# syguan96/DynaBOA

Hardware: AMD Instinct MI355X
Metric: adapted frames/sec, whole job (3 inner + 1 outer step, bs=1 per sequence, first-order; synthetic 224x224 stream, no 3DPW assets in the image: PA-MPJPE on 3DPW not measured) (higher is better)
Workload: dtype f32

## Files before the change

### dynaboa_amd/csrc/adapt_step.hip

```cpp
#include <math.h>
#include <stdlib.h>
#include <string.h>

#include <algorithm>
#include <atomic>
#include <chrono>
#include <condition_variable>
#include <mutex>
#include <string>
#include <thread>
#include <vector>

#include "dyb_common.h"

extern "C" {
size_t dyb_hmr_param_floats(const void*);
size_t dyb_hmr_act_floats(const void*);
size_t dyb_hmr_workspace_bytes(const void*);
int dyb_hmr_forward_train(void*, const float*, const float*, const float*, int, float*, void*, size_t, unsigned long long, unsigned long long, float,
                          hipStream_t);
long long dyb_hmr_act_offset_rotmat(const void*);
long long dyb_hmr_act_offset_state(const void*);
size_t dyb_lbs_saved_floats(int);
size_t dyb_lbs_bwd_workspace_bytes(int);
// ... 233 lines not shown
  bool adam_prepared = false;
  float pre_ss[DYB_MAX_REPLICAS], pre_bc[DYB_MAX_REPLICAS];
  float *gt_rot = nullptr, *gt_verts[3] = {}, *gt_joints = nullptr, *gt_saved = nullptr, *gt17[2] = {};
  DybEvents* ev = nullptr;
  hipEvent_t e_theta = nullptr, e_side = nullptr, e_gt = nullptr;
  int upd_overlap = 1;
  int par_passes = 1, par_max_replicas = DYB_MAX_REPLICAS;
  hipStream_t par_stream[2] = {nullptr, nullptr};
  hipEvent_t par_ev[8] = {nullptr, nullptr, nullptr, nullptr, nullptr, nullptr, nullptr, nullptr};
  bool out_in_main = false;
  int share_dyn_fwd = 1;
  int upd_blocks = 0;
  hipEvent_t e_upd = nullptr;
  DybFwdGates gates{};
  bool gates_pending = false;
  int upd_late = 1;
  struct LateUpd {
    Stepper* S = nullptr;
    bool adam = false, ema = false;
    const float *g2 = nullptr, *g3 = nullptr;
    const float* p = nullptr;
    float* out = nullptr;
    hipStream_t aux = nullptr;
    DybRep scope{};
    float ss[DYB_MAX_REPLICAS], bc[DYB_MAX_REPLICAS];
  } late;
  size_t grp_bounds[2] = {0, 0};
  bool side_pending = false;
  struct Tail {
    bool on = false;
// ... 108 lines not shown
  Stepper* S = new Stepper();
  S->plan = plan; S->B = B; S->H = H; S->W = W;
  S->n_params = dyb_hmr_param_floats(plan);
  S->act_floats = dyb_hmr_act_floats(plan);
  S->ws_bytes = dyb_hmr_workspace_bytes(plan);
  S->off_rot = (size_t)dyb_hmr_act_offset_rotmat(plan);
  S->off_state = (size_t)dyb_hmr_act_offset_state(plan);
  S->lbs_saved = dyb_lbs_saved_floats(B);
  S->lbs_wsb = dyb_lbs_bwd_workspace_bytes(B);
  S->ev = dyb_hmr_events_create(plan);
  dyb_hmr_param_groups(plan, S->grp_bounds);
  if (const char* e = getenv("DYB_UPD_OVERLAP")) S->upd_overlap = atoi(e);
  if (const char* e = getenv("DYB_UPD_BLOCKS")) S->upd_blocks = atoi(e);
  if (const char* e = getenv("DYB_SHARE_DYN_FWD")) S->share_dyn_fwd = atoi(e);
  if (const char* e = getenv("DYB_UPD_LATE")) S->upd_late = atoi(e);
  if (const char* e = getenv("DYB_FUSE_FAST")) S->fuse_fast = atoi(e);
  if (const char* e = getenv("DYB_FUSE_ADAM")) S->fuse_adam = atoi(e);
  if (const char* e = getenv("DYB_FUSE_EMA")) S->fuse_ema = atoi(e);
  if (const char* e = getenv("DYB_PAR_PASSES")) S->par_passes = atoi(e);
  if (const char* e = getenv("DYB_PAR_MAX_REPLICAS")) S->par_max_replicas = atoi(e);
  if (!S->ev || hipEventCreateWithFlags(&S->e_theta, hipEventDisableTiming) != hipSuccess ||
      hipEventCreateWithFlags(&S->e_side, hipEventDisableTiming) != hipSuccess ||
      hipEventCreateWithFlags(&S->e_gt, hipEventDisableTiming) != hipSuccess ||
      hipEventCreateWithFlags(&S->e_upd, hipEventDisableTiming) != hipSuccess ||
      hipEventCreateWithFlags(&S->gates.ev[0], hipEventDisableTiming) != hipSuccess ||
      hipEventCreateWithFlags(&S->gates.ev[1], hipEventDisableTiming) != hipSuccess ||
      hipEventCreateWithFlags(&S->gates.mid, hipEventDisableTiming) != hipSuccess) {
    delete S;
    return DYB_ERR_LAUNCH;
  }
  *out = S;
  return DYB_OK;
}
extern "C" void dyb_stepper_destroy(void* stepper) {
  Stepper* S = reinterpret_cast<Stepper*>(stepper);
  if (!S) return;
  side_shutdown(*S);
  dyb_hmr_events_destroy(S->ev);
  if (S->e_theta) (void)hipEventDestroy(S->e_theta);
  if (S->e_side) (void)hipEventDestroy(S->e_side);
  if (S->e_gt) (void)hipEventDestroy(S->e_gt);
  if (S->e_upd) (void)hipEventDestroy(S->e_upd);
// ... 8 lines not shown
extern "C" int dyb_stepper_set_i(void* stepper, const char* key, long long v) {
  Stepper* S = reinterpret_cast<Stepper*>(stepper);
  DYB_REQUIRE(S && key, DYB_ERR_ARG);
  const std::string k(key);
  if (k == "n_iter") S->n_iter = (int)v;
  else if (k == "inner_step") S->inner_step = (int)v;
  else if (k == "eval_lower") S->eval_lower = (int)v;
  else if (k == "use_side") S->use_side = (int)v;
  else if (k == "upd_overlap") S->upd_overlap = (int)v;
  else if (k == "side_thread") S->side_thread = (int)v;
  else if (k == "upd_blocks") S->upd_blocks = (int)v;
  else if (k == "share_dyn_fwd") S->share_dyn_fwd = (int)v;
  else if (k == "par_passes") S->par_passes = (int)v;
  else if (k == "par_max_replicas") S->par_max_replicas = (int)v;
  else if (k == "upd_late") S->upd_late = (int)v;
  else if (k == "fuse_fast") { DYB_REQUIRE(!S->bound, DYB_ERR_ARG); S->fuse_fast = (int)v; }
  else if (k == "fuse_adam") S->fuse_adam = (int)v;
  else if (k == "fuse_ema") S->fuse_ema = (int)v;
  else if (k == "metrics") S->metrics = (int)v;
  else if (k == "adam_step") {
    S->adam_t = v;
    for (int r = 0; r < DYB_MAX_REPLICAS; ++r) S->adam_t_rep[r] = v;
  }
  else if (k.compare(0, 10, "adam_step_") == 0) {
    const int r = atoi(k.c_str() + 10);
    DYB_REQUIRE(r >= 0 && r < DYB_MAX_REPLICAS, DYB_ERR_ARG);
    S->adam_t_rep[r] = v;
    if (v > S->adam_t) S->adam_t = v;
  }
  else if (k == "full") S->full = (int)v;
// ... 94 lines not shown
  if (k == "loss_floats") return (S->full ? 16 : 4) * (long long)(S->inner_step + 1 + (S->full && S->dynamic ? S->optim_steps : 0));
  if (k == "slots_per_frame") return (S->eval_lower ? S->inner_step : 0) + 1 + (S->full && S->dynamic ? S->optim_steps : 0);
  return -1;
}
extern "C" double dyb_stepper_get_f(const void* stepper, const char* key) {
  const Stepper* S = reinterpret_cast<const Stepper*>(stepper);
  if (!S || !key) return -1.0;
  const std::string k(key);
  if (k == "host_ms_forward") return S->h_fwd;
  if (k == "host_ms_backward") return S->h_bwd;
  if (k == "host_ms_head") return S->h_head;
  if (k == "host_ms_update") return S->h_update;
  if (k == "host_ms_tail") return S->h_tail;
  if (k == "host_ms_total") return S->h_total;
  if (k == "host_frames") return (double)S->h_frames;
  return -1.0;
}
extern "C" size_t dyb_stepper_workspace_bytes(void* stepper) {
  Stepper* S = reinterpret_cast<Stepper*>(stepper);
  if (!S) return 0;
  Stepper tmp = *S;
  return a64(carve(tmp, nullptr) / 4) * 4 * (size_t)S->nrep;
}
extern "C" int dyb_stepper_bind_workspace(void* stepper, void* ws, size_t bytes, hipStream_t st) {
  Stepper* S = reinterpret_cast<Stepper*>(stepper);
  DYB_REQUIRE(S && ws, DYB_ERR_ARG);
  S->blob = a64(carve(*S, nullptr) / 4) * 4;
  DYB_REQUIRE(bytes >= S->blob * (size_t)S->nrep, DYB_ERR_WORKSPACE);
  S->wsp = reinterpret_cast<char*>(ws);
  S->wsp_bytes = bytes;
// ... 39 lines not shown
    }
  }
  DYB_REQUIRE(S.inner_step >= 0 && S.inner_step <= 16 && S.n_iter >= 1 && S.n_iter <= 3, DYB_ERR_UNSUPPORTED);
  return DYB_OK;
}

static int settle_update(Stepper& S, hipStream_t st);
static int pass_forward(Stepper& S, Pass& P, const float* theta, const float* image, hipStream_t st, bool chain = true) {
  const DybFwdGates* gates = (chain && S.gates_pending) ? &S.gates : nullptr;
  {
    const int rc = dyb_hmr_forward_plain(S.plan, theta, image, S.init_state, S.n_iter, P.acts, P.ws, S.ws_bytes, st, gates);
    if (rc != DYB_OK) {
      if (gates) (void)settle_update(S, st);
      return rc;
    }
    if (gates) { DYB_REQUIRE(!S.gates.late, DYB_ERR_LAUNCH); S.gates_pending = false; }
  }
  const float* rot = P.acts + S.off_rot;
  const float* state = P.acts + S.off_state;
  return dyb_lbs_fwd(S.smpl_f[0], S.smpl_i[0], state + 144, STATE_LD, rot, P.verts, P.joints, P.saved, S.B, st);
}
static int pass_frame_head(Stepper& S, Pass& P, const float* kp2d, hipStream_t st) {
  const float* rot = P.acts + S.off_rot;
  const float* state = P.acts + S.off_state;
  return dyb_frame_losses(rot, state + 144, STATE_LD, state + 154, STATE_LD, P.joints, kp2d, S.gmm_means, S.gmm_prec, S.gmm_logw,
                          (float)S.w2d, (float)S.wshape, (float)S.wpose, P.losses, P.drot_l, P.dshape_l, 10, P.dcam_l, 3, P.djoints_l,
                          S.B, P.lws, (size_t)S.B * 16, st);
}
static int pass_backward(Stepper& S, Pass& P, const float* theta, float* grads, hipStream_t st, hipStream_t aux) {
  RUN(dyb_scale_add(nullptr, P.djoints_l, nullptr, P.djoints, (size_t)S.B * NJ * 3, st));
  RUN(dyb_lbs_bwd(S.smpl_f[0], S.smpl_i[0], P.acts + S.off_rot, P.saved, P.djoints, nullptr, P.drot_s, P.dbetas_s, 10, S.B, P.lbs_ws,
                  S.lbs_wsb, st));
  RUN(dyb_head_grad_combine(nullptr, P.drot_l, P.drot_s, nullptr, P.dshape_l, P.dbetas_s, nullptr, P.dcam_l, nullptr, P.d_rot,
                            P.d_state, S.B, st));
  return dyb_hmr_backward_ev(S.plan, theta, P.acts, P.d_rot, P.d_state, S.n_iter, grads, P.ws, S.ws_bytes, st, aux, S.ev);
}
static int gt_meshes(Stepper& S, const float* gt_pose, const float* gt_betas, hipStream_t st) {
  RUN(dyb_rodrigues_fwd(gt_pose, S.gt_rot, S.B * 24, st));
  for (int g = 0; g < 3; ++g)
    RUN(dyb_lbs_fwd(S.smpl_f[g], S.smpl_i[g], gt_betas, 10, S.gt_rot, S.gt_verts[g], S.gt_joints, S.gt_saved, S.B, st));
  RUN(dyb_regress_joints(S.j_h36m, S.gt_verts[1], S.gt17[0], 17, S.B, st));
  return dyb_regress_joints(S.j_h36m, S.gt_verts[2], S.gt17[1], 17, S.B, st);
}
static int record_metrics(Stepper& S, Pass& P, const long long* gender, int slot, hipStream_t st) {
  DYB_REQUIRE(slot >= 0 && slot < S.record_capacity, DYB_ERR_ARG);
  RUN(dyb_regress_joints(S.j_h36m, P.verts, P.pred17, 17, S.B, st));
  float* rec = S.records + (size_t)slot * a64((size_t)S.B * 85 + 1);
  const DybRep& Rp = dyb_rep_current();
  hipLaunchKernelGGL(metric_record_kernel, dim3(1, 1, Rp.n), dim3(256), 0, st, P.pred17, S.gt17[0], S.gt17[1], gender, S.j14, P.verts,
                     S.gt_verts[0], rec, S.B, Rp);
// ... 201 lines not shown
      const double t = (double)(++S.adam_t_rep[r]);
      ss[r] = (float)(S.lr / (1.0 - pow(S.beta1, t)));
      bc[r] = (float)sqrt(1.0 - pow(S.beta2, t));
      if (S.adam_t_rep[r] > S.adam_t) S.adam_t = S.adam_t_rep[r];
    }
  }
  auto range = [&](size_t lo, size_t hi, hipStream_t s) -> int {
    if (adam) {
      const bool fe = ema && S.fuse_ema;
      RUN(adam_range(S, g2, g3, ss, bc, lo, hi, s, fe));
      if (ema && !fe) RUN(dyb_ema_update(S.teacher + lo, S.theta + lo, (float)S.alpha, hi - lo, s));
      return DYB_OK;
    }
    return fastweight_range(S, p, out, g2, g3, lo, hi, s);
  };
  const bool ranged = S.upd_overlap && S.nrep > 1 && aux && aux != st && S.grp_bounds[0] > 0 && S.grp_bounds[1] > S.grp_bounds[0] &&
                      S.grp_bounds[1] < S.n_params;
  if (!ranged) return range(0, S.n_params, st);
  RUN(range(0, S.grp_bounds[0], st));
  HIPOK(hipEventRecord(S.e_upd, st));
  HIPOK(hipStreamWaitEvent(aux, S.e_upd, 0));
  {
    DybStreamCapScope cap(S.upd_blocks > 0 ? (S.upd_blocks / R.n > 0 ? S.upd_blocks / R.n : 1) : 0);
    RUN(range(S.grp_bounds[0], S.grp_bounds[1], aux));
    HIPOK(hipEventRecord(S.gates.ev[0], aux));
    if (S.upd_late) {
      S.late.S = &S; S.late.adam = adam; S.late.ema = ema; S.late.p = p; S.late.out = out; S.late.aux = aux; S.late.scope = R;
      S.late.g2 = g2; S.late.g3 = g3;
      for (int r = 0; r < DYB_MAX_REPLICAS; ++r) { S.late.ss[r] = ss[r]; S.late.bc[r] = bc[r]; }
      S.gates.late = &late_update;
      S.gates.user = &S;
    } else {
      S.gates.late = nullptr;
      RUN(range(S.grp_bounds[1], S.n_params, aux));
      HIPOK(hipEventRecord(S.gates.ev[1], aux));
    }
  }
  S.gates_pending = true;
  return DYB_OK;
}
static int settle_update(Stepper& S, hipStream_t st) {
  if (!S.gates_pending) return DYB_OK;
  if (S.gates.late) {
    HIPOK(hipEventRecord(S.gates.mid, st));
    RUN(late_update(&S));
  }
  HIPOK(hipStreamWaitEvent(st, S.gates.ev[0], 0));
  HIPOK(hipStreamWaitEvent(st, S.gates.ev[1], 0));
  S.gates_pending = false;
  return DYB_OK;
}
static int adam_scope(Stepper& S, hipStream_t st) { return weight_update(S, true, nullptr, nullptr, st, nullptr); }
static int adapt_frame_impl(Stepper& S, const float* image, const float* kp2d, const float* gt_pose, const float* gt_betas,
                            const long long* gender, int record_slot, int loss_slot, hipStream_t st, hipStream_t aux,
                            hipStream_t side) {
  const bool metrics = S.metrics != 0;
  DYB_REQUIRE(!metrics || (gt_pose && gt_betas && gender), DYB_ERR_ARG);
  S.out_in_main = false;
  if (!S.use_side || side == st) side = nullptr;
  const int K = S.inner_step;
  const size_t n = S.n_params;
  float* losslog = (S.loss_log && loss_slot >= 0 && loss_slot < S.loss_capacity) ? S.loss_log + (size_t)loss_slot * 4 * (K + 1) : nullptr;
  int slot = record_slot;
// ... 74 lines not shown
  RUN(pass_forward(S, S.fin, S.theta, image, st));
  RUN(settle_update(S, st));
  if (metrics) RUN(record_metrics(S, S.fin, gender, slot++, st));
  return DYB_OK;
}
static int pass_backward_ext(Stepper& S, Pass& P, const float* theta, float* grads, bool frame_loss, const float* e_rot,
                             const float* e_shape, const float* e_cam, const float* e_joints, hipStream_t st, hipStream_t aux) {
  const size_t nj = (size_t)S.B * NJ * 3;
  if (frame_loss) RUN(dyb_scale_add(nullptr, P.djoints_l, e_joints, P.djoints, nj, st));
  else RUN(dyb_scale_add(nullptr, e_joints, nullptr, P.djoints, nj, st));
  RUN(dyb_lbs_bwd(S.smpl_f[0], S.smpl_i[0], P.acts + S.off_rot, P.saved, P.djoints, nullptr, P.drot_s, P.dbetas_s, 10, S.B, P.lbs_ws,
                  S.lbs_wsb, st));
  const float* z = S.zeros;
  RUN(dyb_head_grad_combine(nullptr, frame_loss ? P.drot_l : z, P.drot_s, e_rot, frame_loss ? P.dshape_l : z, P.dbetas_s, e_shape,
                            frame_loss ? P.dcam_l : z, e_cam, P.d_rot, P.d_state, S.B, st));
  return dyb_hmr_backward_ev(S.plan, theta, P.acts, P.d_rot, P.d_state, S.n_iter, grads, P.ws, S.ws_bytes, st, aux, S.ev);
}
enum { IN_IMAGE = 0, IN_KP, IN_GT_POSE, IN_GT_BETAS, IN_GENDER, IN_HIST_IMAGE, IN_HIST_KP, IN_EX_IMG, IN_EX_KP, IN_EX_POSE,
       IN_EX_BETAS, IN_EX_POSE3D, IN_COUNT };
static int stage_inputs(Stepper& S, const void* const* src, int ld, int k0, int nk, hipStream_t st);
struct FullCtx {
  const void* in[IN_COUNT];
  float* losslog;
  int level_row;
};
struct ParTailGuard {
  hipStream_t st, sB, sC;
  hipEvent_t eB, eC;
  bool armed;
  ~ParTailGuard() {
    if (!armed) return;
// ... 21 lines not shown
    sB = S.par_stream[0]; sC = S.par_stream[1];
    HIPOK(hipEventRecord(S.par_ev[0], st));
    if (motion) HIPOK(hipStreamWaitEvent(sB, S.par_ev[0], 0));
    if (label) HIPOK(hipStreamWaitEvent(sC, S.par_ev[0], 0));
  }
  ParTailGuard tails{st, sB, sC, S.par_ev[6], S.par_ev[7], par};
  if (!have_fwd) RUN(pass_forward(S, P, cur, image, st));
  RUN(pass_frame_head(S, P, kp, st));
  const float* rot = P.acts + S.off_rot;
  const float* state = P.acts + S.off_state;
  if (ranged_before) {
    DYB_REQUIRE(!S.gates_pending && !S.gates.late, DYB_ERR_LAUNCH);
    for (int k = 0; k < 2; ++k) {
      if (motion) HIPOK(hipStreamWaitEvent(sB, S.gates.ev[k], 0));
      if (label) HIPOK(hipStreamWaitEvent(sC, S.gates.ev[k], 0));
    }
  }
  if (par && motion) {
    RUN(pass_forward(S, S.hist, cur, (const float*)C.in[IN_HIST_IMAGE], sB, false));
    HIPOK(hipEventRecord(S.par_ev[1], sB));
  }
  auto label_pass_forward_and_term = [&](hipStream_t s, bool chain) -> int {
    RUN(pass_forward(S, S.ex, cur, (const float*)C.in[IN_EX_IMG], s, chain));
    RUN(dyb_rodrigues_fwd((const float*)C.in[IN_EX_POSE], S.ex_rot, B * 24, s));
    const float* es = S.ex.acts + S.off_state;
    return dyb_aux_loss_terms(2, B, 0, (float)S.label_w, S.ex.acts + S.off_rot, es + 144, STATE_LD, es + 154, STATE_LD, S.ex.joints, nullptr,
                              nullptr, 0, nullptr, 0, nullptr, (const float*)C.in[IN_EX_KP], nullptr, S.ex_rot,
                              (const float*)C.in[IN_EX_BETAS], (const float*)C.in[IN_EX_POSE3D], S.vals_l, S.exg_rot, S.exg_shape, S.exg_cam,
                              S.exg_joints, nullptr, nullptr, s);
  };
// ... 341 lines not shown
  if (S.side_pending) HIPOK(hipStreamWaitEvent(gst, S.e_side, 0));
  RUN(stage_inputs(S, inputs, n, IN_IMAGE, 5, gst));
  const bool have_gt = inputs[2 * n + act[0]] && inputs[3 * n + act[0]] && inputs[4 * n + act[0]];
  if (S.use_side && side && side != st) {
    HIPOK(hipEventRecord(S.e_gt, st));
    HIPOK(hipStreamWaitEvent(side, S.e_gt, 0));
  }
  return adapt_frame_impl(S, S.in_stage[0], S.in_stage[1], have_gt ? S.in_stage[2] : nullptr, have_gt ? S.in_stage[3] : nullptr,
                          have_gt ? reinterpret_cast<const long long*>(S.in_stage[4]) : nullptr, record_slot, loss_slot, st, aux, side);
}
extern "C" int dyb_stepper_join(void* stepper, hipStream_t st) {
  Stepper* S = reinterpret_cast<Stepper*>(stepper);
  DYB_REQUIRE(S, DYB_ERR_ARG);
  RUN(side_wait(*S));
  if ((S->tail.on || S->gtjob.on) && S->tail_stream) RUN(issue_side_work(*S, S->tail_stream));
  if (S->side_pending) {
    HIPOK(hipStreamWaitEvent(st, S->e_side, 0));
    S->side_pending = false;
  }
  return DYB_OK;
}
extern "C" const float* dyb_stepper_output(const void* stepper, int which) {
  const Stepper* S = reinterpret_cast<const Stepper*>(stepper);
  if (!S || !S->bound) return nullptr;
  const Pass& F = (S->out_in_main ? S->main : S->fin);
  switch (which) {
    case 0: return F.acts + S->off_rot;
    case 1: return F.acts + S->off_state;
    case 2: return F.verts;
    case 3: return F.joints;
// ... 4 lines not shown
```

### dynaboa_amd/csrc/dyb_common.h

```cpp
#pragma once
#if defined(__HIP_DEVICE_COMPILE__) && !defined(__gfx950__)
#error "libdynaboa_hip is written for gfx950 (MI355X) only"
#endif
#include <hip/hip_runtime.h>
#include <stdint.h>

#include <vector>
#include "dyb_switches.h"

#define DYB_OK 0
#define DYB_ERR_ARG (-1)
#define DYB_ERR_LAUNCH (-2)
#define DYB_ERR_UNSUPPORTED (-3)
#define DYB_ERR_WORKSPACE (-4)

#define DYB_GN_GROUPS 4
#define DYB_GN_EPS 1e-5f

#define DYB_CHECK_LAUNCH()                                  \
  do {                                                      \
    if (hipGetLastError() != hipSuccess) return DYB_ERR_LAUNCH; \
  } while (0)

#define DYB_REQUIRE(cond, code) \
// ... 217 lines not shown
                       const float* stats, const float* gamma, const float* beta, float* dm, float* dy, float* dgamma, float* dbeta,
                       int HW, int C, int relu, int k, float* part, unsigned* ctr, hipStream_t st);
int dyb_zero_words(unsigned* p, int n, hipStream_t st);
int dyb_gn_bwd_apply_dy(const float* dm, const float* y, const float* stats, const float* part, int nch, int ncolb,
                        const float* gamma, float* dy, float* dgamma, float* dbeta, int N, int HW, int C, hipStream_t st);
int dyb_conv_dgrad_plain_raw(const ConvDesc& d, const float* dy, const float* w, float* dx, const float* addend, void* ws,
                             size_t ws_bytes, int* nslabs, hipStream_t st);
int dyb_conv_wgrad_plain(const ConvDesc& d, const float* x, const float* y_prev, const float* stats_prev, const float* gamma_prev,
                         const float* beta_prev, const float* dy, float* dw, void* ws, size_t ws_bytes, hipStream_t st);
int dyb_avgpool_fwd_tail(const float* x, float* const* dsts, int ndst, int ld, int N, int HW, int C, const float* tail,
                         int tail_ld, int tail_cols, int tail_dst_col, hipStream_t st);

struct DybEvents {
  std::vector<hipEvent_t> dy;
  hipEvent_t join = nullptr;
};
DybEvents* dyb_hmr_events_create(const void* plan);
void dyb_hmr_events_destroy(DybEvents* e);
struct DybFwdGates {
  hipEvent_t ev[2];
  hipEvent_t mid = nullptr;
  int (*late)(void* user) = nullptr;
  void* user = nullptr;
};
void dyb_hmr_param_groups(const void* plan, size_t bounds[2]);
int dyb_hmr_forward_plain(void* plan, const float* params, const float* image, const float* init_state, int n_iter, float* acts,
                          void* ws, size_t ws_bytes, hipStream_t st, const DybFwdGates* gates = nullptr);
int dyb_hmr_backward_ev(void* plan, const float* params, const float* acts, const float* d_rotmat, const float* d_state,
                        int n_iter, float* grads, void* ws, size_t ws_bytes, hipStream_t st, hipStream_t aux, const DybEvents* ev);
```

### dynaboa_amd/csrc/hmr_engine.hip

```cpp
#include <stdlib.h>
#include <string.h>

#include <mutex>
#include <string>
#include <unordered_map>
#include <vector>

#include "dyb_common.h"

extern "C" {
size_t dyb_conv2d_workspace_bytes(int, int, int, int, int, int, int, int, int);
size_t dyb_groupnorm_workspace_bytes(int, int, int);
int dyb_conv2d_nhwc_fwd_gnstats(const float*, const float*, int, const float*, const float*, int, float*, const float*, float*,
                                float*, int*, int, int, int, int, int, int, int, int, int, void*, size_t, hipStream_t);
int dyb_groupnorm_apply_n(const float*, const float*, int, const float*, const float*, const float*, const float*, int,
                          const float*, const float*, float*, float*, float*, int, int, int, int, hipStream_t);
int dyb_conv2d_nhwc_wgrad_gn_n(const float*, const float*, const float*, const float*, const float*, const float*, const float*,
                               const float*, const float*, int, int, const float*, float*, float*, float*, int, int, int, int,
                               int, int, int, int, int, void*, size_t, hipStream_t);
size_t dyb_groupnorm_bwd_partial_floats(int, int, int);
int dyb_conv2d_nhwc_dgrad_gn(const float*, const float*, const float*, const float*, const float*, const float*, float*,
                             const float*, int, int, int, int, int, int, int, int, int, void*, size_t, hipStream_t);
int dyb_conv2d_nhwc_wgrad_gn(const float*, const float*, const float*, const float*, const float*, const float*, float*,
                             float*, float*, int, int, int, int, int, int, int, int, int, void*, size_t, hipStream_t);
// ... 248 lines not shown
  RUN_RC(fill_events(P, P.ev));
  P.events_ready = true;
  return DYB_OK;
}
DybEvents* dyb_hmr_events_create(const void* plan) {
  const HmrPlan* P = reinterpret_cast<const HmrPlan*>(plan);
  if (!P) return nullptr;
  DybEvents* e = new DybEvents();
  if (fill_events(*P, *e) != DYB_OK) { delete e; return nullptr; }
  return e;
}
void dyb_hmr_events_destroy(DybEvents* e) {
  if (!e) return;
  for (hipEvent_t x : e->dy) (void)hipEventDestroy(x);
  (void)hipEventDestroy(e->join);
  delete e;
}
extern "C" size_t dyb_hmr_param_floats(const void* plan) { return reinterpret_cast<const HmrPlan*>(plan)->n_params; }
extern "C" size_t dyb_hmr_act_floats(const void* plan) { return reinterpret_cast<const HmrPlan*>(plan)->act_floats; }
extern "C" size_t dyb_hmr_workspace_bytes(const void* plan) { return reinterpret_cast<const HmrPlan*>(plan)->ws_total; }
extern "C" int dyb_hmr_num_tensors(const void* plan) { return (int)reinterpret_cast<const HmrPlan*>(plan)->tensors.size(); }
extern "C" int dyb_hmr_tensor_info(const void* plan, int i, char* name, int name_cap, int* kind, long long* offset,
                                   int* dims4, int* cin_pad) {
  const HmrPlan* P = reinterpret_cast<const HmrPlan*>(plan);
  DYB_REQUIRE(P && i >= 0 && i < (int)P->tensors.size() && name && kind && offset && dims4 && cin_pad, DYB_ERR_ARG);
  const TensorInfo& t = P->tensors[i];
  strncpy(name, t.name.c_str(), name_cap - 1);
  name[name_cap - 1] = 0;
  *kind = t.kind; *offset = (long long)t.offset; *cin_pad = t.cin_pad;
  for (int k = 0; k < 4; ++k) dims4[k] = t.dims[k];
// ... 210 lines not shown
                            nullptr, nullptr, acts + stem.out, acts + stem.stats, B, stem.Ho * stem.Wo, stem.K, 1, st));
  RUN(dyb_maxpool3x3s2_fwd(acts + stem.out, acts + P.a_pool, reinterpret_cast<uint32_t*>(acts + P.a_poolidx), B, stem.Ho,
                           stem.Wo, stem.K, st));
  const float* x = acts + P.a_pool;
  for (int bi = 0; bi < (int)P.blocks.size(); ++bi) {
    const BlockL& b = P.blocks[bi];
    const ConvL &c1 = P.convs[b.c1], &c2 = P.convs[b.c2], &c3 = P.convs[b.c3];
    if (gates) {
      if (bi == P.layer_last_block[1] + 1) {
        if (gates->ev[0] && hipStreamWaitEvent(st, gates->ev[0], 0) != hipSuccess) return DYB_ERR_LAUNCH;
        if (gates->late) {
          if (gates->mid && hipEventRecord(gates->mid, st) != hipSuccess) return DYB_ERR_LAUNCH;
          RUN(gates->late(gates->user));
        }
      }
      if (bi == P.layer_last_block[2] + 1 && gates->ev[1] && hipStreamWaitEvent(st, gates->ev[1], 0) != hipSuccess) return DYB_ERR_LAUNCH;
    }
    RUN(conv_stats(P, c1, params, acts, x, nullptr, nullptr, 0, w.gn[0], &nA, w, st));
    RUN(conv_stats(P, c2, params, acts, nullptr, &c1, w.gn[0], nA, w.gn[1], &nB, w, st));
    if (b.cd >= 0) RUN(conv_stats(P, P.convs[b.cd], params, acts, x, nullptr, nullptr, 0, w.gn[2], &nD, w, st));
    RUN(conv_stats(P, c3, params, acts, nullptr, &c2, w.gn[1], nB, w.gn[0], &nA, w, st));
    if (b.cd >= 0) {
      const ConvL& cd = P.convs[b.cd];
      RUN(dyb_groupnorm_apply_n(acts + c3.y, w.gn[0], nA, params + c3.gam, params + c3.bet, acts + cd.y, w.gn[2], nD,
                                params + cd.gam, params + cd.bet, acts + cd.stats, acts + c3.out, acts + c3.stats, B,
                                c3.Ho * c3.Wo, c3.K, 1, st));
    } else {
      RUN(dyb_groupnorm_apply_n(acts + c3.y, w.gn[0], nA, params + c3.gam, params + c3.bet, x, nullptr, 0, nullptr, nullptr,
                                nullptr, acts + c3.out, acts + c3.stats, B, c3.Ho * c3.Wo, c3.K, 1, st));
    }
    x = acts + c3.out;
  }
  float* dsts[MAX_ITER];
  for (int t = 0; t < n_iter; ++t) dsts[t] = acts + P.a_xc[t];
  RUN(dyb_avgpool_fwd_tail(x, dsts, n_iter, FC1_IN_PAD, B, P.featHW, FEAT, init_state, STATE_LD, STATE_LD, FEAT, st));
  float* fc1_pre = reinterpret_cast<float*>(w.lin);
  RUN(dyb_linear_fwd(acts + P.a_xc[0], FC1_IN_PAD, params + P.fc1_w, FC1_IN_PAD, params + P.fc1_b, nullptr, 0, fc1_pre, HID, B, FEAT, HID, st));
  for (int t = 0; t < n_iter; ++t) {
    const float* xc = acts + P.a_xc[t];
    RUN(dyb_linear_fwd(xc + FEAT, FC1_IN_PAD, params + P.fc1_w + FEAT, FC1_IN_PAD, nullptr, fc1_pre, HID, acts + P.a_h1[t], HID, B,
                       FC1_IN_PAD - FEAT, HID, st));
    const float* h1 = acts + P.a_h1[t];
    if (drop.on) {
      RUN(dropout_launch(h1, acts + P.a_h1d[t], B * HID, drop, 2u * t, st));
      h1 = acts + P.a_h1d[t];
    }
    RUN(dyb_linear_fwd(h1, HID, params + P.fc2_w, HID, params + P.fc2_b, nullptr, 0, acts + P.a_h2[t], HID, B, HID, HID, st));
    const float* h2 = acts + P.a_h2[t];
    if (drop.on) {
// ... 75 lines not shown
                              acts + c.stats, params + c.gam, params + c.bet, dm, part, P.B, c.Ho * c.Wo, c.K, relu, st,
                              tp ? nullptr : done));
  if (tp) {
    float* dyl = w.dy2 + c.dy;
    RUN(dyb_gn_bwd_apply_dy(dm, acts + c.y, acts + c.stats, part, 0, 0, params + c.gam, dyl, grads + c.gam, grads + c.bet, P.B,
                            c.Ho * c.Wo, c.K, st));
    if (done && hipEventRecord(done, st) != hipSuccess) return DYB_ERR_LAUNCH;
    j.dy = dyl;
  }
  if (jobs) jobs->push_back(j);
  else RUN(run_wgrad(P, j, params, acts, grads, w, w.conv, st));
  *dm_out = dm;
  return DYB_OK;
}
static int flush_wgrads(HmrPlan& P, std::vector<WgradJob>& jobs, hipEvent_t done, const float* params, const float* acts,
                        float* grads, const WsCarve& w, hipStream_t aux) {
  if (hipStreamWaitEvent(aux, done, 0) != hipSuccess) return DYB_ERR_LAUNCH;
  for (const WgradJob& j : jobs) RUN(run_wgrad(P, j, params, acts, grads, w, w.conv_aux, aux));
  jobs.clear();
  return DYB_OK;
}
static int layer_dgrad(HmrPlan& P, int ci, const float* params, const float* acts, const float* dm, float* dx_buf,
                       const float* addend, Pending* out, const WsCarve& w, hipStream_t st, const BwdState& bs) {
  const ConvL& c = P.convs[ci];
  ConvDesc d{P.B, c.H, c.W, c.C, c.K, c.R, c.S, c.stride, c.pad};
  GnBwdSrc src{dm, acts + c.y, acts + c.stats, w.gnb + c.gnb, params + c.gam, bs.nch[ci], bs.ncolb[ci]};
  int ns = 1;
  if (dyb_throughput_mode(P.B))
    RUN(dyb_conv_dgrad_plain_raw(d, w.dy2 + c.dy, params + c.w, dx_buf, addend, w.conv, P.ws_conv,
                                 (out && P.fold_in_reduce) ? &ns : nullptr, st));
  else
    RUN(dyb_conv_dgrad_gn_raw(d, src, params + c.w, dx_buf, addend, w.conv, P.ws_conv, (out && P.fold_in_reduce) ? &ns : nullptr,
                              st));
// ... 10 lines not shown
  ConvDesc d{P.B, c.H, c.W, c.C, c.K, c.R, c.S, c.stride, c.pad};
  *done = false;
  if (!dyb_conv_dgrad_k4_ok(d)) return DYB_OK;
  GnBwdSrc src{dm, acts + c.y, acts + c.stats, w.gnb + c.gnb, params + c.gam, bs.nch[ci], bs.ncolb[ci]};
  int nch = 0, ncolb = 0;
  RUN(dyb_conv_dgrad_k4(d, src, params + c.w, addend, acts + p.y, p.has_out ? acts + p.out : nullptr, acts + p.stats,
                        params + p.gam, params + p.bet, w.dy + p.dy, w.gnb + p.gnb, &nch, &ncolb, st, nullptr));
  bs.nch[pi] = nch; bs.ncolb[pi] = ncolb; bs.reduced[pi] = 1;
  *dm_p = w.dy + p.dy;
  *done = true;
  return DYB_OK;
}

static int backward_body(HmrPlan& P, const float* params, const float* acts, const float* d_rotmat, const float* d_state,
                         int n_iter, float* grads, const WsCarve& w, hipStream_t st, hipStream_t aux, const DybEvents& E,
                         const DropCfg& drop = kNoDrop);

int dyb_hmr_backward_ev(void* plan, const float* params, const float* acts, const float* d_rotmat, const float* d_state,
                        int n_iter, float* grads, void* ws, size_t ws_bytes, hipStream_t st, hipStream_t aux, const DybEvents* ev) {
  HmrPlan* Pp = reinterpret_cast<HmrPlan*>(plan);
  DYB_REQUIRE(Pp && params && acts && d_rotmat && d_state && grads && ws, DYB_ERR_ARG);
  DYB_REQUIRE(n_iter >= 1 && n_iter <= MAX_ITER, DYB_ERR_UNSUPPORTED);
  DYB_REQUIRE(ws_bytes >= Pp->ws_total, DYB_ERR_WORKSPACE);
  if (aux == st || !ev) aux = nullptr;
  WsCarve w = carve(*Pp, ws);
  static const DybEvents none;
  return backward_body(*Pp, params, acts, d_rotmat, d_state, n_iter, grads, w, st, aux, ev ? *ev : none);
}
void dyb_hmr_param_groups(const void* plan, size_t bounds[2]) {
  const HmrPlan* P = reinterpret_cast<const HmrPlan*>(plan);
  bounds[0] = P->convs[P->blocks[P->layer_last_block[1] + 1].c1].w;
  bounds[1] = P->convs[P->blocks[P->layer_last_block[2] + 1].c1].w;
}
int dyb_hmr_forward_plain(void* plan, const float* params, const float* image, const float* init_state, int n_iter, float* acts,
                          void* ws, size_t ws_bytes, hipStream_t st, const DybFwdGates* gates) {
  HmrPlan* Pp = reinterpret_cast<HmrPlan*>(plan);
  DYB_REQUIRE(Pp && params && image && init_state && acts && ws, DYB_ERR_ARG);
  DYB_REQUIRE(n_iter >= 1 && n_iter <= MAX_ITER, DYB_ERR_UNSUPPORTED);
  DYB_REQUIRE(ws_bytes >= Pp->ws_total && Pp->featHW == 49, DYB_ERR_WORKSPACE);
  WsCarve w = carve(*Pp, ws);
  RUN(dyb_nchw3_to_nhwc4(image, acts + Pp->a_x4, Pp->B, Pp->H, Pp->W, st));
  return forward_body(*Pp, params, init_state, n_iter, acts, w, st, kNoDrop, gates);
// ... 32 lines not shown
  DYB_REQUIRE(Pp && params && acts && d_rotmat && d_state && grads && ws, DYB_ERR_ARG);
  DYB_REQUIRE(n_iter >= 1 && n_iter <= MAX_ITER, DYB_ERR_UNSUPPORTED);
  HmrPlan& P = *Pp;
  DYB_REQUIRE(ws_bytes >= P.ws_total, DYB_ERR_WORKSPACE);
  if (aux == st) aux = nullptr;
  if (aux) RUN(ensure_events(P));
  WsCarve w = carve(P, ws);
  GKey key{{(uintptr_t)params, (uintptr_t)acts, (uintptr_t)d_rotmat, (uintptr_t)d_state, (uintptr_t)grads, (uintptr_t)ws,
            (uintptr_t)st, (uintptr_t)aux, (uintptr_t)n_iter, 0}};
  return run_cached(P, P.gbwd, key, st,
                    [&]() { return backward_body(P, params, acts, d_rotmat, d_state, n_iter, grads, w, st, aux, P.ev); });
}

static int backward_body(HmrPlan& P, const float* params, const float* acts, const float* d_rotmat, const float* d_state,
                         int n_iter, float* grads, const WsCarve& w, hipStream_t st, hipStream_t aux, const DybEvents& E,
                         const DropCfg& drop) {
  DybBf16Scope bf(P.bf16 != 0);
  const int B = P.B;
  float* d_st[MAX_ITER + 1];
  float *d_h2[MAX_ITER], *d_h1[MAX_ITER];
  float* r = w.reg;
  for (int t = 0; t <= MAX_ITER; ++t) { d_st[t] = r; r += (size_t)B * STATE_LD; }
  for (int t = 0; t < MAX_ITER; ++t) { d_h2[t] = r; r += (size_t)B * HID; }
  for (int t = 0; t < MAX_ITER; ++t) { d_h1[t] = r; r += (size_t)B * HID; }
  float* d_xf = r;

  RUN(dyb_scale_add(nullptr, d_state, nullptr, d_st[n_iter], (size_t)B * STATE_LD, st));
  RUN(dyb_rot6d_bwd(acts + P.a_state, STATE_LD, d_rotmat, d_st[n_iter], STATE_LD, B, st));
  for (int t = n_iter - 1; t >= 0; --t) {
    RUN(dyb_linear_bwd_dx(d_st[t + 1], STATE_LD, params + P.dec_w, HID, B, HID, STATE_LD, d_h2[t], HID, 0, HID, nullptr, 0,
                          nullptr, 0, w.lin, P.ws_lin, st));
// ... 3 lines not shown
    if (drop.on) RUN(dropout_launch(d_h1[t], d_h1[t], B * HID, drop, 2u * t, st));
    RUN(dyb_linear_bwd_dx(d_h1[t], HID, params + P.fc1_w + FEAT, FC1_IN_PAD, B, FC1_IN_PAD - FEAT, HID, d_st[t], STATE_LD, 0, 0, d_st[t],
                          STATE_LD, d_st[t + 1], STATE_LD, w.lin, P.ws_lin, st));
  }
  {
    float* sbuf[2] = {d_xf + (size_t)B * FC1_IN_PAD, d_xf + (size_t)B * (FC1_IN_PAD + HID)};
    const float* dsum = d_h1[0];
    for (int t = 1; t < n_iter; ++t) {
      float* o = sbuf[t & 1];
      RUN(dyb_scale_add(nullptr, dsum, d_h1[t], o, (size_t)B * HID, st));
      dsum = o;
    }
    RUN(dyb_linear_bwd_dx(dsum, HID, params + P.fc1_w, FC1_IN_PAD, B, FEAT, HID, d_xf, FC1_IN_PAD, 0, FEAT, nullptr, 0, nullptr, 0, w.lin,
                          P.ws_lin, st));
  }
  {
    const float *dys[MAX_ITER], *xs[MAX_ITER];
    int ldd[MAX_ITER], ldx[MAX_ITER];
    for (int t = 0; t < n_iter; ++t) { dys[t] = d_st[t + 1]; ldd[t] = STATE_LD; xs[t] = acts + (drop.on ? P.a_h2d[t] : P.a_h2[t]); ldx[t] = HID; }
    RUN(dyb_linear_bwd_dw(dys, ldd, xs, ldx, n_iter, B, HID, STATE_LD, grads + P.dec_w, HID, grads + P.dec_b, st));
    for (int t = 0; t < n_iter; ++t) { dys[t] = d_h2[t]; ldd[t] = HID; xs[t] = acts + (drop.on ? P.a_h1d[t] : P.a_h1[t]); ldx[t] = HID; }
    RUN(dyb_linear_bwd_dw(dys, ldd, xs, ldx, n_iter, B, HID, HID, grads + P.fc2_w, HID, grads + P.fc2_b, st));
    for (int t = 0; t < n_iter; ++t) { dys[t] = d_h1[t]; ldd[t] = HID; xs[t] = acts + P.a_xc[t]; ldx[t] = FC1_IN_PAD; }
    RUN(dyb_linear_bwd_dw(dys, ldd, xs, ldx, n_iter, B, FC1_IN_PAD, HID, grads + P.fc1_w, FC1_IN_PAD, grads + P.fc1_b, st));
  }

  float *D0 = w.g[0], *D1 = w.g[1], *Rb = w.g[2];
  RUN(dyb_zero_words(w.sync, (int)(align64(P.convs.size() * SYNC_WORDS) + 2 * DYB_CONV_SYNC_WORDS), st));
  DybConvSyncScope conv_sync(conv_ctr(P, w, 0), DYB_CONV_SYNC_WORDS);
  RUN(dyb_avgpool_bwd(d_xf, FC1_IN_PAD, D0, B, P.featHW, FEAT, st));
  Pending cur = plain(D0);
  float* free_buf = D1;
  std::vector<WgradJob> jobs_store;
  std::vector<WgradJob>* jobs = aux ? &jobs_store : nullptr;
  BwdState bs;
  bs.nch.assign(P.convs.size(), 0); bs.ncolb.assign(P.convs.size(), 0); bs.reduced.assign(P.convs.size(), 0);
  auto push_wgrad = [&](int ci, const float* conv_in, const ConvL* in_prev, const float* dm) -> int {
    WgradJob j{ci, conv_in, in_prev, dm, bs.nch[ci], bs.ncolb[ci], nullptr};
    if (jobs) { jobs->push_back(j); return DYB_OK; }
    return run_wgrad(P, j, params, acts, grads, w, w.conv, st);
// ... 13 lines not shown
    } else {
      RUN(layer_gn_bwd(P, b.c3, params, acts, grads, nullptr, &c2, cur, 1, &dm3, w, st, jobs, nullptr));
    }
    RUN(layer_dgrad_k4(P, b.c3, b.c2, params, acts, dm3, nullptr, w, st, bs, &dm2, &k4));
    if (k4) {
      RUN(push_wgrad(b.c2, nullptr, &c1, dm2));
    } else {
      RUN(layer_dgrad(P, b.c3, params, acts, dm3, free_buf, nullptr, &p3, w, st, bs));
      RUN(layer_gn_bwd(P, b.c2, params, acts, grads, nullptr, &c1, p3, 1, &dm2, w, st, jobs, nullptr, false));
    }
    RUN(layer_dgrad(P, b.c2, params, acts, dm2, other, nullptr, &p2, w, st, bs));
    const float* edge = dm3;
    if (b.cd >= 0) {
      RUN(layer_gn_bwd(P, b.c1, params, acts, grads, xin, nullptr, p2, 1, &dm1, w, st, jobs, nullptr, false));
      RUN(layer_gn_bwd(P, b.cd, params, acts, grads, xin, nullptr, plain(dm3), 0, &dmd, w, st, jobs, ev, false));
      if (aux) RUN(flush_wgrads(P, jobs_store, ev, params, acts, grads, w, aux));
      RUN(layer_dgrad(P, b.cd, params, acts, dmd, Rb, nullptr, nullptr, w, st, bs));
      edge = Rb;
    } else {
      RUN(layer_gn_bwd(P, b.c1, params, acts, grads, xin, nullptr, p2, 1, &dm1, w, st, jobs, ev, false));
      if (aux) RUN(flush_wgrads(P, jobs_store, ev, params, acts, grads, w, aux));
    }
    k4 = false;
    if (bi > 0) {
      const float* dmp = nullptr;
      RUN(layer_dgrad_k4(P, b.c1, P.blocks[bi - 1].c3, params, acts, dm1, edge, w, st, bs, &dmp, &k4));
    }
    if (!k4) {
      RUN(layer_dgrad(P, b.c1, params, acts, dm1, free_buf, edge, &pout, w, st, bs));
      cur = pout;
      if (cur.nslabs == 1) free_buf = other;
    }
  }
  const ConvL& stem = P.convs[0];
  const float* gpool = cur.base;
  float* spare = free_buf;
  if (cur.nslabs > 1) {
    RUN(dyb_splitk_fold(cur.base, cur.nslabs, (size_t)B * P.poolH * P.poolW * stem.K, cur.addend, free_buf, st));
    gpool = free_buf;
    spare = (free_buf == D0) ? D1 : D0;
  }
  RUN(dyb_maxpool3x3s2_bwd(gpool, reinterpret_cast<const uint32_t*>(acts + P.a_poolidx), spare, B, stem.Ho, stem.Wo, stem.K, st));
  const float* dm0;
  RUN(layer_gn_bwd(P, 0, params, acts, grads, acts + P.a_x4, nullptr, plain(spare), 1, &dm0, w, st, jobs,
                   aux ? E.dy[0] : nullptr, false));
  if (aux) RUN(flush_wgrads(P, jobs_store, E.dy[0], params, acts, grads, w, aux));
  if (aux) {
    if (hipEventRecord(E.join, aux) != hipSuccess) return DYB_ERR_LAUNCH;
    if (hipStreamWaitEvent(st, E.join, 0) != hipSuccess) return DYB_ERR_LAUNCH;
  }
  return DYB_OK;
}

#include "hvp_engine.inc"
```

Before: 491.6.

## Defer layer4 and regressor weight-grads to aux stream past backward join

```diff
diff --git a/dynaboa_amd/csrc/adapt_step.hip b/dynaboa_amd/csrc/adapt_step.hip
--- a/dynaboa_amd/csrc/adapt_step.hip
+++ b/dynaboa_amd/csrc/adapt_step.hip
@@ -271,6 +271,9 @@
   hipEvent_t e_upd = nullptr;
   DybFwdGates gates{};
   bool gates_pending = false;
+  int wgrad_defer = 1;
+  bool defer_pending = false;
+  int n_deferred = 0;
   int upd_late = 1;
   struct LateUpd {
     Stepper* S = nullptr;
@@ -409,6 +412,7 @@
   if (const char* e = getenv("DYB_UPD_BLOCKS")) S->upd_blocks = atoi(e);
   if (const char* e = getenv("DYB_SHARE_DYN_FWD")) S->share_dyn_fwd = atoi(e);
   if (const char* e = getenv("DYB_UPD_LATE")) S->upd_late = atoi(e);
+  if (const char* e = getenv("DYB_WGRAD_DEFER")) S->wgrad_defer = atoi(e);
   if (const char* e = getenv("DYB_FUSE_FAST")) S->fuse_fast = atoi(e);
   if (const char* e = getenv("DYB_FUSE_ADAM")) S->fuse_adam = atoi(e);
   if (const char* e = getenv("DYB_FUSE_EMA")) S->fuse_ema = atoi(e);
@@ -420,7 +424,9 @@
       hipEventCreateWithFlags(&S->e_upd, hipEventDisableTiming) != hipSuccess ||
       hipEventCreateWithFlags(&S->gates.ev[0], hipEventDisableTiming) != hipSuccess ||
       hipEventCreateWithFlags(&S->gates.ev[1], hipEventDisableTiming) != hipSuccess ||
-      hipEventCreateWithFlags(&S->gates.mid, hipEventDisableTiming) != hipSuccess) {
+      hipEventCreateWithFlags(&S->gates.mid, hipEventDisableTiming) != hipSuccess ||
+      hipEventCreateWithFlags(&S->ev->l4, hipEventDisableTiming) != hipSuccess ||
+      hipEventCreateWithFlags(&S->ev->reg, hipEventDisableTiming) != hipSuccess) {
     delete S;
     return DYB_ERR_LAUNCH;
   }
@@ -459,6 +465,7 @@
   else if (k == "par_passes") S->par_passes = (int)v;
   else if (k == "par_max_replicas") S->par_max_replicas = (int)v;
   else if (k == "upd_late") S->upd_late = (int)v;
+  else if (k == "wgrad_defer") S->wgrad_defer = (int)v;
   else if (k == "fuse_fast") { DYB_REQUIRE(!S->bound, DYB_ERR_ARG); S->fuse_fast = (int)v; }
   else if (k == "fuse_adam") S->fuse_adam = (int)v;
   else if (k == "fuse_ema") S->fuse_ema = (int)v;
@@ -583,6 +590,7 @@
   if (k == "host_ms_tail") return S->h_tail;
   if (k == "host_ms_total") return S->h_total;
   if (k == "host_frames") return (double)S->h_frames;
+  if (k == "deferred_launches") return (double)S->n_deferred;
   return -1.0;
 }
 extern "C" size_t dyb_stepper_workspace_bytes(void* stepper) {
@@ -652,7 +660,7 @@
       if (gates) (void)settle_update(S, st);
       return rc;
     }
-    if (gates) { DYB_REQUIRE(!S.gates.late, DYB_ERR_LAUNCH); S.gates_pending = false; }
+    if (gates) { DYB_REQUIRE(!S.gates.late, DYB_ERR_LAUNCH); S.gates_pending = false; S.defer_pending = false; }
   }
   const float* rot = P.acts + S.off_rot;
   const float* state = P.acts + S.off_state;
@@ -665,13 +673,22 @@
                           (float)S.w2d, (float)S.wshape, (float)S.wpose, P.losses, P.drot_l, P.dshape_l, 10, P.dcam_l, 3, P.djoints_l,
                           S.B, P.lws, (size_t)S.B * 16, st);
 }
+static bool ranged_form(const Stepper& S, hipStream_t st, hipStream_t aux) {
+  return S.upd_overlap && S.nrep > 1 && aux && aux != st && S.grp_bounds[0] > 0 && S.grp_bounds[1] > S.grp_bounds[0] &&
+         S.grp_bounds[1] < S.n_params;
+}
+static int engine_backward(Stepper& S, Pass& P, const float* theta, float* grads, hipStream_t st, hipStream_t aux) {
+  const bool defer = S.wgrad_defer && ranged_form(S, st, aux) && S.ev->l4 && S.ev->reg;
+  if (defer) S.defer_pending = true;
+  return dyb_hmr_backward_ev(S.plan, theta, P.acts, P.d_rot, P.d_state, S.n_iter, grads, P.ws, S.ws_bytes, st, aux, S.ev, defer, &S.n_deferred);
+}
 static int pass_backward(Stepper& S, Pass& P, const float* theta, float* grads, hipStream_t st, hipStream_t aux) {
   RUN(dyb_scale_add(nullptr, P.djoints_l, nullptr, P.djoints, (size_t)S.B * NJ * 3, st));
   RUN(dyb_lbs_bwd(S.smpl_f[0], S.smpl_i[0], P.acts + S.off_rot, P.saved, P.djoints, nullptr, P.drot_s, P.dbetas_s, 10, S.B, P.lbs_ws,
                   S.lbs_wsb, st));
   RUN(dyb_head_grad_combine(nullptr, P.drot_l, P.drot_s, nullptr, P.dshape_l, P.dbetas_s, nullptr, P.dcam_l, nullptr, P.d_rot,
                             P.d_state, S.B, st));
-  return dyb_hmr_backward_ev(S.plan, theta, P.acts, P.d_rot, P.d_state, S.n_iter, grads, P.ws, S.ws_bytes, st, aux, S.ev);
+  return engine_backward(S, P, theta, grads, st, aux);
 }
 static int gt_meshes(Stepper& S, const float* gt_pose, const float* gt_betas, hipStream_t st) {
   RUN(dyb_rodrigues_fwd(gt_pose, S.gt_rot, S.B * 24, st));
@@ -903,9 +920,17 @@
     }
     return fastweight_range(S, p, out, g2, g3, lo, hi, s);
   };
-  const bool ranged = S.upd_overlap && S.nrep > 1 && aux && aux != st && S.grp_bounds[0] > 0 && S.grp_bounds[1] > S.grp_bounds[0] &&
-                      S.grp_bounds[1] < S.n_params;
-  if (!ranged) return range(0, S.n_params, st);
+  const bool ranged = ranged_form(S, st, aux);
+  if (!ranged) {
+    if (S.defer_pending) {
+      HIPOK(hipStreamWaitEvent(st, S.ev->l4, 0));
+      HIPOK(hipStreamWaitEvent(st, S.ev->reg, 0));
+      S.defer_pending = false;
+    }
+    return range(0, S.n_params, st);
+  }
+  S.gates.l4 = S.defer_pending ? S.ev->l4 : nullptr;
+  S.gates.reg = S.defer_pending ? S.ev->reg : nullptr;
   RUN(range(0, S.grp_bounds[0], st));
   HIPOK(hipEventRecord(S.e_upd, st));
   HIPOK(hipStreamWaitEvent(aux, S.e_upd, 0));
@@ -929,6 +954,11 @@
   return DYB_OK;
 }
 static int settle_update(Stepper& S, hipStream_t st) {
+  if (S.defer_pending && !S.gates_pending) {
+    HIPOK(hipStreamWaitEvent(st, S.ev->l4, 0));
+    HIPOK(hipStreamWaitEvent(st, S.ev->reg, 0));
+    S.defer_pending = false;
+  }
   if (!S.gates_pending) return DYB_OK;
   if (S.gates.late) {
     HIPOK(hipEventRecord(S.gates.mid, st));
@@ -936,6 +966,11 @@
   }
   HIPOK(hipStreamWaitEvent(st, S.gates.ev[0], 0));
   HIPOK(hipStreamWaitEvent(st, S.gates.ev[1], 0));
+  if (S.defer_pending) {
+    HIPOK(hipStreamWaitEvent(st, S.ev->l4, 0));
+    HIPOK(hipStreamWaitEvent(st, S.ev->reg, 0));
+    S.defer_pending = false;
+  }
   S.gates_pending = false;
   return DYB_OK;
 }
@@ -1040,7 +1075,7 @@
   const float* z = S.zeros;
   RUN(dyb_head_grad_combine(nullptr, frame_loss ? P.drot_l : z, P.drot_s, e_rot, frame_loss ? P.dshape_l : z, P.dbetas_s, e_shape,
                             frame_loss ? P.dcam_l : z, e_cam, P.d_rot, P.d_state, S.B, st));
-  return dyb_hmr_backward_ev(S.plan, theta, P.acts, P.d_rot, P.d_state, S.n_iter, grads, P.ws, S.ws_bytes, st, aux, S.ev);
+  return engine_backward(S, P, theta, grads, st, aux);
 }
 enum { IN_IMAGE = 0, IN_KP, IN_GT_POSE, IN_GT_BETAS, IN_GENDER, IN_HIST_IMAGE, IN_HIST_KP, IN_EX_IMG, IN_EX_KP, IN_EX_POSE,
        IN_EX_BETAS, IN_EX_POSE3D, IN_COUNT };
@@ -1092,6 +1127,10 @@
     for (int k = 0; k < 2; ++k) {
       if (motion) HIPOK(hipStreamWaitEvent(sB, S.gates.ev[k], 0));
       if (label) HIPOK(hipStreamWaitEvent(sC, S.gates.ev[k], 0));
+    }
+    for (hipEvent_t e : {S.gates.l4, S.gates.reg}) {
+      if (e && motion) HIPOK(hipStreamWaitEvent(sB, e, 0));
+      if (e && label) HIPOK(hipStreamWaitEvent(sC, e, 0));
     }
   }
   if (par && motion) {
@@ -1463,6 +1502,7 @@
   DYB_REQUIRE(S, DYB_ERR_ARG);
   RUN(side_wait(*S));
   if ((S->tail.on || S->gtjob.on) && S->tail_stream) RUN(issue_side_work(*S, S->tail_stream));
+  if (S->defer_pending && !S->gates_pending) RUN(settle_update(*S, st));
   if (S->side_pending) {
     HIPOK(hipStreamWaitEvent(st, S->e_side, 0));
     S->side_pending = false;
diff --git a/dynaboa_amd/csrc/dyb_common.h b/dynaboa_amd/csrc/dyb_common.h
--- a/dynaboa_amd/csrc/dyb_common.h
+++ b/dynaboa_amd/csrc/dyb_common.h
@@ -255,6 +255,7 @@
 struct DybEvents {
   std::vector<hipEvent_t> dy;
   hipEvent_t join = nullptr;
+  hipEvent_t l4 = nullptr, reg = nullptr;
 };
 DybEvents* dyb_hmr_events_create(const void* plan);
 void dyb_hmr_events_destroy(DybEvents* e);
@@ -263,9 +264,11 @@
   hipEvent_t mid = nullptr;
   int (*late)(void* user) = nullptr;
   void* user = nullptr;
+  hipEvent_t l4 = nullptr, reg = nullptr;
 };
 void dyb_hmr_param_groups(const void* plan, size_t bounds[2]);
 int dyb_hmr_forward_plain(void* plan, const float* params, const float* image, const float* init_state, int n_iter, float* acts,
                           void* ws, size_t ws_bytes, hipStream_t st, const DybFwdGates* gates = nullptr);
 int dyb_hmr_backward_ev(void* plan, const float* params, const float* acts, const float* d_rotmat, const float* d_state,
-                        int n_iter, float* grads, void* ws, size_t ws_bytes, hipStream_t st, hipStream_t aux, const DybEvents* ev);
+                        int n_iter, float* grads, void* ws, size_t ws_bytes, hipStream_t st, hipStream_t aux, const DybEvents* ev,
+                        bool defer = false, int* n_deferred = nullptr);
diff --git a/dynaboa_amd/csrc/hmr_engine.hip b/dynaboa_amd/csrc/hmr_engine.hip
--- a/dynaboa_amd/csrc/hmr_engine.hip
+++ b/dynaboa_amd/csrc/hmr_engine.hip
@@ -286,6 +286,8 @@
   if (!e) return;
   for (hipEvent_t x : e->dy) (void)hipEventDestroy(x);
   (void)hipEventDestroy(e->join);
+  if (e->l4) (void)hipEventDestroy(e->l4);
+  if (e->reg) (void)hipEventDestroy(e->reg);
   delete e;
 }
 extern "C" size_t dyb_hmr_param_floats(const void* plan) { return reinterpret_cast<const HmrPlan*>(plan)->n_params; }
@@ -526,7 +528,10 @@
           RUN(gates->late(gates->user));
         }
       }
-      if (bi == P.layer_last_block[2] + 1 && gates->ev[1] && hipStreamWaitEvent(st, gates->ev[1], 0) != hipSuccess) return DYB_ERR_LAUNCH;
+      if (bi == P.layer_last_block[2] + 1) {
+        if (gates->ev[1] && hipStreamWaitEvent(st, gates->ev[1], 0) != hipSuccess) return DYB_ERR_LAUNCH;
+        if (gates->l4 && hipStreamWaitEvent(st, gates->l4, 0) != hipSuccess) return DYB_ERR_LAUNCH;
+      }
     }
     RUN(conv_stats(P, c1, params, acts, x, nullptr, nullptr, 0, w.gn[0], &nA, w, st));
     RUN(conv_stats(P, c2, params, acts, nullptr, &c1, w.gn[0], nA, w.gn[1], &nB, w, st));
@@ -545,6 +550,7 @@
   }
   float* dsts[MAX_ITER];
   for (int t = 0; t < n_iter; ++t) dsts[t] = acts + P.a_xc[t];
+  if (gates && gates->reg && hipStreamWaitEvent(st, gates->reg, 0) != hipSuccess) return DYB_ERR_LAUNCH;
   RUN(dyb_avgpool_fwd_tail(x, dsts, n_iter, FC1_IN_PAD, B, P.featHW, FEAT, init_state, STATE_LD, STATE_LD, FEAT, st));
   float* fc1_pre = reinterpret_cast<float*>(w.lin);
   RUN(dyb_linear_fwd(acts + P.a_xc[0], FC1_IN_PAD, params + P.fc1_w, FC1_IN_PAD, params + P.fc1_b, nullptr, 0, fc1_pre, HID, B, FEAT, HID, st));
@@ -650,9 +656,13 @@
   return DYB_OK;
 }
 static int flush_wgrads(HmrPlan& P, std::vector<WgradJob>& jobs, hipEvent_t done, const float* params, const float* acts,
-                        float* grads, const WsCarve& w, hipStream_t aux) {
+                        float* grads, const WsCarve& w, hipStream_t aux, const std::vector<char>& deferrable,
+                        std::vector<WgradJob>& held) {
   if (hipStreamWaitEvent(aux, done, 0) != hipSuccess) return DYB_ERR_LAUNCH;
-  for (const WgradJob& j : jobs) RUN(run_wgrad(P, j, params, acts, grads, w, w.conv_aux, aux));
+  for (const WgradJob& j : jobs) {
+    if (deferrable[j.ci] && j.dy) held.push_back(j);
+    else RUN(run_wgrad(P, j, params, acts, grads, w, w.conv_aux, aux));
+  }
   jobs.clear();
   return DYB_OK;
 }
@@ -693,10 +703,11 @@
 
 static int backward_body(HmrPlan& P, const float* params, const float* acts, const float* d_rotmat, const float* d_state,
                          int n_iter, float* grads, const WsCarve& w, hipStream_t st, hipStream_t aux, const DybEvents& E,
-                         const DropCfg& drop = kNoDrop);
+                         const DropCfg& drop = kNoDrop, bool defer_req = false, int* n_deferred = nullptr);
 
 int dyb_hmr_backward_ev(void* plan, const float* params, const float* acts, const float* d_rotmat, const float* d_state,
-                        int n_iter, float* grads, void* ws, size_t ws_bytes, hipStream_t st, hipStream_t aux, const DybEvents* ev) {
+                        int n_iter, float* grads, void* ws, size_t ws_bytes, hipStream_t st, hipStream_t aux, const DybEvents* ev,
+                        bool defer, int* n_deferred) {
   HmrPlan* Pp = reinterpret_cast<HmrPlan*>(plan);
   DYB_REQUIRE(Pp && params && acts && d_rotmat && d_state && grads && ws, DYB_ERR_ARG);
   DYB_REQUIRE(n_iter >= 1 && n_iter <= MAX_ITER, DYB_ERR_UNSUPPORTED);
@@ -704,7 +715,7 @@
   if (aux == st || !ev) aux = nullptr;
   WsCarve w = carve(*Pp, ws);
   static const DybEvents none;
-  return backward_body(*Pp, params, acts, d_rotmat, d_state, n_iter, grads, w, st, aux, ev ? *ev : none);
+  return backward_body(*Pp, params, acts, d_rotmat, d_state, n_iter, grads, w, st, aux, ev ? *ev : none, kNoDrop, defer, n_deferred);
 }
 void dyb_hmr_param_groups(const void* plan, size_t bounds[2]) {
   const HmrPlan* P = reinterpret_cast<const HmrPlan*>(plan);
@@ -767,7 +778,7 @@
 
 static int backward_body(HmrPlan& P, const float* params, const float* acts, const float* d_rotmat, const float* d_state,
                          int n_iter, float* grads, const WsCarve& w, hipStream_t st, hipStream_t aux, const DybEvents& E,
-                         const DropCfg& drop) {
+                         const DropCfg& drop, bool defer_req, int* n_deferred) {
   DybBf16Scope bf(P.bf16 != 0);
   const int B = P.B;
   float* d_st[MAX_ITER + 1];
@@ -801,16 +812,28 @@
     RUN(dyb_linear_bwd_dx(dsum, HID, params + P.fc1_w, FC1_IN_PAD, B, FEAT, HID, d_xf, FC1_IN_PAD, 0, FEAT, nullptr, 0, nullptr, 0, w.lin,
                           P.ws_lin, st));
   }
-  {
+  auto regressor_dw = [&](hipStream_t s) -> int {
     const float *dys[MAX_ITER], *xs[MAX_ITER];
     int ldd[MAX_ITER], ldx[MAX_ITER];
     for (int t = 0; t < n_iter; ++t) { dys[t] = d_st[t + 1]; ldd[t] = STATE_LD; xs[t] = acts + (drop.on ? P.a_h2d[t] : P.a_h2[t]); ldx[t] = HID; }
-    RUN(dyb_linear_bwd_dw(dys, ldd, xs, ldx, n_iter, B, HID, STATE_LD, grads + P.dec_w, HID, grads + P.dec_b, st));
+    RUN(dyb_linear_bwd_dw(dys, ldd, xs, ldx, n_iter, B, HID, STATE_LD, grads + P.dec_w, HID, grads + P.dec_b, s));
     for (int t = 0; t < n_iter; ++t) { dys[t] = d_h2[t]; ldd[t] = HID; xs[t] = acts + (drop.on ? P.a_h1d[t] : P.a_h1[t]); ldx[t] = HID; }
-    RUN(dyb_linear_bwd_dw(dys, ldd, xs, ldx, n_iter, B, HID, HID, grads + P.fc2_w, HID, grads + P.fc2_b, st));
+    RUN(dyb_linear_bwd_dw(dys, ldd, xs, ldx, n_iter, B, HID, HID, grads + P.fc2_w, HID, grads + P.fc2_b, s));
     for (int t = 0; t < n_iter; ++t) { dys[t] = d_h1[t]; ldd[t] = HID; xs[t] = acts + P.a_xc[t]; ldx[t] = FC1_IN_PAD; }
-    RUN(dyb_linear_bwd_dw(dys, ldd, xs, ldx, n_iter, B, FC1_IN_PAD, HID, grads + P.fc1_w, FC1_IN_PAD, grads + P.fc1_b, st));
-  }
+    return dyb_linear_bwd_dw(dys, ldd, xs, ldx, n_iter, B, FC1_IN_PAD, HID, grads + P.fc1_w, FC1_IN_PAD, grads + P.fc1_b, s);
+  };
+  const bool defer = aux && defer_req && E.l4 && E.reg && !drop.on;
+  std::vector<char> deferrable(P.convs.size(), 0);
+  if (defer) {
+    const int first4 = P.layer_last_block[2] + 1;
+    for (int bi = first4; bi < (int)P.blocks.size(); ++bi) {
+      const BlockL& b = P.blocks[bi];
+      deferrable[b.c2] = deferrable[b.c3] = 1;
+      if (bi > first4) deferrable[b.c1] = 1;
+    }
+  }
+  std::vector<WgradJob> deferred;
+  if (!defer) RUN(regressor_dw(st));
 
   float *D0 = w.g[0], *D1 = w.g[1], *Rb = w.g[2];
   RUN(dyb_zero_words(w.sync, (int)(align64(P.convs.size() * SYNC_WORDS) + 2 * DYB_CONV_SYNC_WORDS), st));
@@ -854,12 +877,12 @@
     if (b.cd >= 0) {
       RUN(layer_gn_bwd(P, b.c1, params, acts, grads, xin, nullptr, p2, 1, &dm1, w, st, jobs, nullptr, false));
       RUN(layer_gn_bwd(P, b.cd, params, acts, grads, xin, nullptr, plain(dm3), 0, &dmd, w, st, jobs, ev, false));
-      if (aux) RUN(flush_wgrads(P, jobs_store, ev, params, acts, grads, w, aux));
+      if (aux) RUN(flush_wgrads(P, jobs_store, ev, params, acts, grads, w, aux, deferrable, deferred));
       RUN(layer_dgrad(P, b.cd, params, acts, dmd, Rb, nullptr, nullptr, w, st, bs));
       edge = Rb;
     } else {
       RUN(layer_gn_bwd(P, b.c1, params, acts, grads, xin, nullptr, p2, 1, &dm1, w, st, jobs, ev, false));
-      if (aux) RUN(flush_wgrads(P, jobs_store, ev, params, acts, grads, w, aux));
+      if (aux) RUN(flush_wgrads(P, jobs_store, ev, params, acts, grads, w, aux, deferrable, deferred));
     }
     k4 = false;
     if (bi > 0) {
@@ -884,10 +907,17 @@
   const float* dm0;
   RUN(layer_gn_bwd(P, 0, params, acts, grads, acts + P.a_x4, nullptr, plain(spare), 1, &dm0, w, st, jobs,
                    aux ? E.dy[0] : nullptr, false));
-  if (aux) RUN(flush_wgrads(P, jobs_store, E.dy[0], params, acts, grads, w, aux));
+  if (aux) RUN(flush_wgrads(P, jobs_store, E.dy[0], params, acts, grads, w, aux, deferrable, deferred));
   if (aux) {
     if (hipEventRecord(E.join, aux) != hipSuccess) return DYB_ERR_LAUNCH;
     if (hipStreamWaitEvent(st, E.join, 0) != hipSuccess) return DYB_ERR_LAUNCH;
+    if (defer) {
+      for (const WgradJob& j : deferred) RUN(run_wgrad(P, j, params, acts, grads, w, w.conv_aux, aux));
+      if (hipEventRecord(E.l4, aux) != hipSuccess) return DYB_ERR_LAUNCH;
+      RUN(regressor_dw(aux));
+      if (hipEventRecord(E.reg, aux) != hipSuccess) return DYB_ERR_LAUNCH;
+      if (n_deferred) *n_deferred += (int)deferred.size() + 3;
+    }
   }
   return DYB_OK;
 }
```

After: 497.2, median of 6. +1.1%, better.
